# bepu/bepuphysics2

Hardware: NVIDIA H100
Metric: constraint-iterations/sec (solver+integrator) (higher is better)
Workload: dtype f32

## Files before the change

### bepuphysics2_b200/csrc/bepu_layout_kernels.h

```cpp
#pragma once
#include "bepu_device_types.h"

namespace bepucuda {

void launch_split_bodies(const void* raw, int body_count, const BodyBuffers& B, cudaStream_t s);
void launch_merge_bodies(void* raw, int body_count, const BodyBuffers& B, cudaStream_t s);
struct TransposeDesc {
    int32_t* src_refs;
    float* src_prestep;
    float* src_impulses;
    const int32_t* map;
    int32_t src_count;
    int32_t bodies, prestep_rows, impulse_rows;
    int32_t src_bundle_base;
    int32_t flags;
    const int32_t* features_old;
    const int32_t* features_new;
};
constexpr int32_t kDescResidentImpulses = 1, kDescRedistribute = 2;
enum { kTransposeRefs = 1, kTransposePrestep = 2, kTransposeImpulses = 4 };
void launch_transpose_in_all(const DeviceTypeBatch* tbs, const TransposeDesc* descs, const WorkItem* work, int work_count, int W, int what, cudaStream_t s);
void launch_transpose_out_all(const DeviceTypeBatch* tbs, const TransposeDesc* descs, const WorkItem* work, int work_count, int W, int what, cudaStream_t s);
void launch_fill_i32(int32_t* p, size_t n, int32_t v, cudaStream_t s);
void launch_redistribute_impulses(const DeviceTypeBatch* tbs, const TransposeDesc* descs, const WorkItem* work, int work_count, cudaStream_t s);
// ... 5 lines not shown
    size_t bytes;
};
void launch_batched_copy(const CopyChunk* chunks, int chunk_count, cudaStream_t s);
void launch_ownership_pass1(const DeviceTypeBatch* tbs, const WorkItem* work, int work_count, const int32_t* bodies_per_type, int sync_batch_count, int body_count,
                            int32_t* first_batch, int32_t* sync_refcount, unsigned long long* sync_mask, int32_t* error_flag, cudaStream_t s);
void launch_ownership_rest(const DeviceTypeBatch* tbs, const WorkItem* work, int work_count, const int32_t* bodies_per_type, int body_count, const int32_t* first_batch,
                           const int32_t* sync_refcount, const unsigned long long* sync_mask, uint8_t* constrained, const int32_t* kinematics, int kinematic_count,
                           int32_t* error_flag, const TransposeDesc* descs, int W, int32_t* source_bundle_flags, cudaStream_t s);
void launch_shard_barrier(const ShardPeers& peers, const FrameParams* fp, uint32_t exchange_index, int32_t* error_flag, cudaStream_t s);

void launch_fill_peer_masks(const int32_t* refs, uint32_t* peer_masks, size_t count, const uint8_t* body_masks, int rank, cudaStream_t s);
void launch_boundary_flags(const WorkRecord* records, int count, const int32_t* bodies_per_type, long long peer_delta, uint8_t* flags, cudaStream_t s);

void launch_pack_ref_rows(const WorkRecord* records, int count, int32_t* rows, cudaStream_t s);

constexpr int kLaunchPdl = 1, kLaunchPrefetchRows = 2, kLaunchIntegratorExtensions = 4;
struct ShardLaunch {
    ShardPeers peers;
    long long peer_delta;
    ShardStage stage;
};
struct SolverLaunchers {
    void (*constraint_stage)(int stage, const WorkRecord* records, const int32_t* ref_rows, int work_count, const BodyBuffers& B, const FrameParams* fp, int launch_flags,
                             const ShardLaunch* shard, cudaStream_t s);
    void (*kinematic_stage)(int stage, const int32_t* kinematics, int count, const BodyBuffers& B, const FrameParams* fp, int launch_flags, cudaStream_t s);
    void (*final_pose)(const BodyBuffers& B, const FrameParams* fp, int launch_flags, cudaStream_t s);
};
const SolverLaunchers* get_launchers_bepu_fast();
const SolverLaunchers* get_launchers_bepu_strict();

}
// ... 1 lines not shown
```

### bepuphysics2_b200/csrc/bepu_solver_kernels.cu

```cuda
#include <atomic>
#include "bepu_solver_kernels.cuh"
#include "bepu_layout_kernels.h"

namespace BEPU_NS {

using StageLauncher = void(const WorkRecord* records, const int32_t* ref_rows, int work_count, const BodyBuffers& B, const FrameParams* fp, int launch_flags,
                           const ShardLaunch* shard, cudaStream_t s);
StageLauncher launch_stage_warm_start_first, launch_stage_warm_start, launch_stage_solve;

#ifndef BEPU_DEEP_MINB
#define BEPU_DEEP_MINB 12
#endif
constexpr int kDeepBatchBundles = 2150;
template <auto Kernel, class... Args>
static void launch_stage_kernel(int work_count, int launch_flags, cudaStream_t s, Args... args) {
    static std::atomic<bool> carveout_set[64] = {};
    int device = 0;
    cudaGetDevice(&device);
    if (!carveout_set[device & 63]) {
        cudaFuncSetAttribute(Kernel, cudaFuncAttributePreferredSharedMemoryCarveout, cudaSharedmemCarveoutMaxShared);
        carveout_set[device & 63] = true;
    }
    const unsigned blocks = (unsigned)(((size_t)work_count * 32 + kStageBlockThreads - 1) / kStageBlockThreads);
    cudaLaunchConfig_t cfg{};
    cfg.gridDim = dim3(blocks);
    cfg.blockDim = dim3(kStageBlockThreads);
    cfg.stream = s;
    cudaLaunchAttribute attr[1];
    attr[0].id = cudaLaunchAttributeProgrammaticStreamSerialization;
    attr[0].val.programmaticStreamSerializationAllowed = 1;
    cfg.attrs = attr;
    cfg.numAttrs = (launch_flags & bepucuda::kLaunchPdl) ? 1 : 0;
    cudaLaunchKernelEx(&cfg, Kernel, args...);
}
template <int STAGE, int MINB, bool kExt>
static void launch_stage_instance(const WorkRecord* records, const int32_t* ref_rows, int work_count, const BodyBuffers& B, const FrameParams* fp, int launch_flags, const ShardLaunch* shard,
                                  cudaStream_t s) {
    const int flags = (launch_flags & bepucuda::kLaunchPrefetchRows) ? kStagePrefetchRows : 0;
    if (!shard) launch_stage_kernel<constraint_stage_kernel<STAGE, MINB, kExt>>(work_count, launch_flags, s, records, ref_rows, work_count, B, fp, flags);
    else if constexpr (STAGE != kStageIncremental)
        launch_stage_kernel<constraint_stage_kernel_sharded<STAGE, MINB, kExt>>(work_count, launch_flags, s, records, ref_rows, work_count, B, fp, flags, shard->peers, shard->peer_delta,
                                                                               shard->stage);
}
template <int STAGE, int MINB>
static void launch_stage_variant(const WorkRecord* records, const int32_t* ref_rows, int work_count, const BodyBuffers& B, const FrameParams* fp, int launch_flags, const ShardLaunch* shard,
                                 cudaStream_t s) {
    if constexpr (STAGE == kStageWarmStartFirst || STAGE == kStageWarmStart) {
        if (launch_flags & bepucuda::kLaunchIntegratorExtensions) return launch_stage_instance<STAGE, MINB, true>(records, ref_rows, work_count, B, fp, launch_flags, shard, s);
    }
    launch_stage_instance<STAGE, MINB, false>(records, ref_rows, work_count, B, fp, launch_flags, shard, s);
}
template <int STAGE>
static void launch_stage_t(const WorkRecord* records, const int32_t* ref_rows, int work_count, const BodyBuffers& B, const FrameParams* fp, int launch_flags, const ShardLaunch* shard, cudaStream_t s) {
    if constexpr (STAGE != kStageIncremental) {
        if (work_count >= kDeepBatchBundles) return launch_stage_variant<STAGE, BEPU_DEEP_MINB>(records, ref_rows, work_count, B, fp, launch_flags, shard, s);
    }
    launch_stage_variant<STAGE, 1>(records, ref_rows, work_count, B, fp, launch_flags, shard, s);
}

#if BEPU_UNIT == 0
void launch_stage_warm_start_first(const WorkRecord* records, const int32_t* ref_rows, int work_count, const BodyBuffers& B, const FrameParams* fp, int launch_flags, const ShardLaunch* shard, cudaStream_t s) {
    launch_stage_t<kStageWarmStartFirst>(records, ref_rows, work_count, B, fp, launch_flags, shard, s);
}
#elif BEPU_UNIT == 1
void launch_stage_warm_start(const WorkRecord* records, const int32_t* ref_rows, int work_count, const BodyBuffers& B, const FrameParams* fp, int launch_flags, const ShardLaunch* shard, cudaStream_t s) {
    launch_stage_t<kStageWarmStart>(records, ref_rows, work_count, B, fp, launch_flags, shard, s);
}
#elif BEPU_UNIT == 2
void launch_stage_solve(const WorkRecord* records, const int32_t* ref_rows, int work_count, const BodyBuffers& B, const FrameParams* fp, int launch_flags, const ShardLaunch* shard, cudaStream_t s) {
    launch_stage_t<kStageSolve>(records, ref_rows, work_count, B, fp, launch_flags, shard, s);
}
#elif BEPU_UNIT == 3
// ... 36 lines not shown
```

### bepuphysics2_b200/csrc/bepu_solver_kernels.cuh

```cuda
#pragma once
#include "bepu_contacts.cuh"
#include "bepu_joints_more.cuh"
#include "bepu_integration.cuh"
#include "bepu_device_types.h"

namespace BEPU_NS {

using namespace bepucuda;

struct F8 { float a, b, c, d, e, f, g, h; };
#define BEPU_BODY_LD "ld.global.L1::no_allocate.L2::cache_hint.v4.f32"
#define BEPU_BODY_ST "st.global.L1::no_allocate.L2::cache_hint.v4.f32"
BEPU_DI uint64_t l2_evict_last_policy() {
    uint64_t policy;
    asm("createpolicy.fractional.L2::evict_last.b64 %0, 1.0;" : "=l"(policy));
    return policy;
}
BEPU_DI F8 ld256(const float4* p) {
    F8 r;
    asm volatile(BEPU_BODY_LD " {%0,%1,%2,%3}, [%8], %9;\n\t" BEPU_BODY_LD " {%4,%5,%6,%7}, [%8+16], %9;"
                 : "=f"(r.a), "=f"(r.b), "=f"(r.c), "=f"(r.d), "=f"(r.e), "=f"(r.f), "=f"(r.g), "=f"(r.h)
                 : "l"(p), "l"(l2_evict_last_policy())
                 : "memory");
    return r;
// ... 29 lines not shown
    if (flags & kIntegrateAccelerations) {
        const F8 a = ld256(accelerations + 2 * (size_t)idx);
        linearAcceleration = {a.a, a.b, a.c};
        angularAcceleration = {a.e, a.f, a.g};
    }
    integrate_velocity_extensions(v, (flags & kIntegrateAccelerations) != 0, linearAcceleration, angularAcceleration, dt, (flags & kIntegratePointGravity) != 0, position, center,
                                  attractorDt);
    return v;
}
BEPU_DI void apply_velocity_extensions(const FrameParams& fp, uint32_t idx, V3 position, float dt, float attractorDt, Velocity& v) {
    const float4* accelerations = reinterpret_cast<const float4*>((unsigned long long)fp.accelerations[0] | ((unsigned long long)fp.accelerations[1] << 32));
    v = integrate_velocity_extensions_at(fp.integrate_extensions, accelerations, idx, v.lin, v.ang, dt, position, V3{fp.attractor_center[0], fp.attractor_center[1], fp.attractor_center[2]},
                                         attractorDt);
}

template <int STAGE, bool NeedsPose, bool kExt>
BEPU_DI void warm_start_body(uint32_t enc, const BodyBuffers& B, const FrameParams& fp, BodyState& b, Velocity& v) {
    const uint32_t idx = enc & kRefIndexMask;
    if (enc & kRefIntegrateBit) {
        Inertia local;
        load_inertia(B.inertia_local, idx, local);
        load_pose(B.pose, idx, b.pos, b.q);
        b.inertia.inv_mass = local.inv_mass;
        if (STAGE == kStageWarmStart) {
            b.pos = b.pos + v.lin * fp.dt;
            Q4 previousOrientation = b.q;
            b.q = integrate_orientation(b.q, v.ang, fp.dt * 0.5f);
            b.inertia.t = rotate_inverse_inertia(local.t, b.q);
            if (fp.angular_mode == 1) integrate_angular_conserve_momentum(previousOrientation, local.t, b.inertia.t, v.ang);
            else if (fp.angular_mode == 2) integrate_angular_gyroscopic(b.q, local.t, v.ang, fp.dt);
            store_pose(B.pose, idx, b.pos, b.q);
        } else {
            b.inertia.t = rotate_inverse_inertia(local.t, b.q);
            if (fp.angular_mode == 1) {
                Q4 previousOrientation = integrate_orientation(b.q, v.ang, fp.dt * -0.5f);
                integrate_angular_conserve_momentum(previousOrientation, local.t, b.inertia.t, v.ang);
            } else if (fp.angular_mode == 2) {
// ... 6 lines not shown
    } else {
        load_inertia(B.inertia_world, idx, b.inertia);
        if (NeedsPose) load_pose(B.pose, idx, b.pos, b.q);
        if (STAGE == kStageWarmStartFirst && fp.angular_mode != 0 && (enc & kRefBundleIntegratesBit) && !(enc & kRefKinematicBit)) {
            Inertia local;
            load_inertia(B.inertia_local, idx, local);
            V3 pos;
            Q4 q;
            load_pose(B.pose, idx, pos, q);
            if (fp.angular_mode == 1) integrate_angular_conserve_momentum(integrate_orientation(q, v.ang, fp.dt * -0.5f), local.t, b.inertia.t, v.ang);
            else integrate_angular_gyroscopic(q, local.t, v.ang, fp.dt);
        }
    }
}
template <int STAGE, bool NeedsPose, bool kExt>
BEPU_DI void gather_for_warm_start(uint32_t enc, const BodyBuffers& B, const FrameParams& fp, BodyState& b, Velocity& v) {
    load_velocity(B.velocity, enc & kRefIndexMask, v);
    warm_start_body<STAGE, NeedsPose, kExt>(enc, B, fp, b, v);
}

template <class T, class PR, class AR> BEPU_DI void call_warm_start(const BodyState* b, PR p, AR a, Velocity* v) {
    if constexpr (T::kNeedsPose) T::warm_start(b, p, a, v);
    else if constexpr (T::kBodies == 2) T::warm_start(b[0].inertia, b[1].inertia, p, a, v[0], v[1]);
    else T::warm_start(b[0].inertia, p, a, v[0]);
}
template <class T, class PR, class AR> BEPU_DI void call_solve(const BodyState* b, float dt, float inverseDt, PR p, AR a, Velocity* v) {
    if constexpr (T::kNeedsPose) T::solve(b, dt, inverseDt, p, a, v);
    else if constexpr (T::kBodies == 2) T::solve(b[0].inertia, b[1].inertia, dt, inverseDt, p, a, v[0], v[1]);
    else T::solve(b[0].inertia, dt, inverseDt, p, a, v[0]);
}
template <class T> BEPU_DI void call_incremental(float dt, const Velocity* v, float* p) {
    if constexpr (T::kIncremental) {
        if constexpr (T::kBodies == 2) T::incremental_update(dt, v[0], v[1], p);
// ... 4 lines not shown
BEPU_DI uint32_t ldg_nc_u32(const void* p) {
    uint32_t v;
    asm volatile("ld.global.nc.u32 %0, [%1];" : "=r"(v) : "l"(p));
    return v;
}
BEPU_DI void push_record(float4* const* arrays, uint32_t mask, uint32_t idx, float a, float b, float c, float d, float e, float f, float g, float h) {
    while (mask) {
        const int q = __ffs((int)mask) - 1;
        mask &= mask - 1u;
        float4* dst = arrays[q] + 2 * (size_t)idx;
        dst[0] = make_float4(a, b, c, d);
        dst[1] = make_float4(e, f, g, h);
    }
}
template <class T, int STAGE, bool kSharded, bool kExt, class PR, class AR>
BEPU_DI void run_lane(const int32_t* refs, PR p, AR a, float* p_rw, uint32_t enc0, uint32_t enc1, const BodyBuffers& B, const FrameParams& fp, const ShardPeers* peers = nullptr,
                      long long peer_delta = 0) {
    constexpr int NB = T::kBodies;
    uint32_t enc[NB];
    enc[0] = enc0;
    if constexpr (NB > 1) enc[1] = enc1;
#pragma unroll
    for (int s = 2; s < NB; ++s) enc[s] = (uint32_t)__ldg(refs + s * kLanes);
    uint32_t push_to[kSharded ? NB : 1];
    if constexpr (kSharded) {
#pragma unroll
        for (int s = 0; s < NB; ++s) push_to[s] = peer_delta != 0 ? ldg_nc_u32(refs + peer_delta + s * kLanes) : 0u;
    }
    if ((int32_t)enc[0] == kRefEmpty) return;
    BodyState b[NB];
    Velocity v[NB];
    if constexpr (STAGE == kStageIncremental) {
#pragma unroll
        for (int s = 0; s < NB; ++s) load_velocity(B.velocity, enc[s] & kRefIndexMask, v[s]);
        call_incremental<T>(fp.dt, v, p_rw);
    } else if constexpr (STAGE == kStageSolve) {
#pragma unroll
        for (int s = 0; s < NB; ++s) {
            const uint32_t idx = enc[s] & kRefIndexMask;
            load_velocity(B.velocity, idx, v[s]);
            load_inertia(B.inertia_world, idx, b[s].inertia);
            if (T::kNeedsPose) load_pose(B.pose, idx, b[s].pos, b[s].q);
        }
        rows_ready(p);
        call_solve<T>(b, fp.dt, fp.inverse_dt, p, a, v);
#pragma unroll
        for (int s = 0; s < NB; ++s)
            if (!(enc[s] & kRefKinematicBit)) {
                store_velocity(B.velocity, enc[s] & kRefIndexMask, v[s]);
                if constexpr (kSharded) {
                    const uint32_t mask = push_to[s];
                    if (mask) push_record(peers->velocity, mask, enc[s] & kRefIndexMask, v[s].lin.x, v[s].lin.y, v[s].lin.z, 0.0f, v[s].ang.x, v[s].ang.y, v[s].ang.z, 0.0f);
                }
            }
    } else {
#pragma unroll
        for (int s = 0; s < NB; ++s) gather_for_warm_start<STAGE, T::kNeedsPose, kExt>(enc[s], B, fp, b[s], v[s]);
        rows_ready(p);
        call_warm_start<T>(b, p, a, v);
#pragma unroll
        for (int s = 0; s < NB; ++s)
            if (!(enc[s] & kRefKinematicBit)) {
                const uint32_t idx = enc[s] & kRefIndexMask;
                store_velocity(B.velocity, idx, v[s]);
                if constexpr (kSharded) {
                    const uint32_t mask = push_to[s];
                    if (mask) {
                        push_record(peers->velocity, mask, idx, v[s].lin.x, v[s].lin.y, v[s].lin.z, 0.0f, v[s].ang.x, v[s].ang.y, v[s].ang.z, 0.0f);
                        if (enc[s] & kRefIntegrateBit) {
                            const Inertia& in = b[s].inertia;
                            push_record(peers->inertia_world, mask, idx, in.t.xx, in.t.yx, in.t.yy, in.t.zx, in.t.zy, in.t.zz, in.inv_mass, 0.0f);
                            if (STAGE == kStageWarmStart) push_record(peers->pose, mask, idx, b[s].q.x, b[s].q.y, b[s].q.z, b[s].q.w, b[s].pos.x, b[s].pos.y, b[s].pos.z, 0.0f);
                        }
                    }
                }
            }
    }
}
template <class T, int STAGE, class PR, class AR>
BEPU_DI void run_lane(const int32_t* refs, PR p, AR a, float* p_rw, uint32_t enc0, uint32_t enc1, const BodyBuffers& B, const FrameParams& fp) {
    run_lane<T, STAGE, false, false>(refs, p, a, p_rw, enc0, enc1, B, fp);
}

BEPU_DI int4 ldg_nc_v4(const void* p) {
    int4 v;
    asm volatile("ld.global.nc.v4.s32 {%0,%1,%2,%3}, [%4];" : "=r"(v.x), "=r"(v.y), "=r"(v.z), "=r"(v.w) : "l"(p));
    return v;
}
BEPU_DI WorkRecord load_record(const WorkRecord* r) {
    const int4 lo = ldg_nc_v4(r), hi = ldg_nc_v4(reinterpret_cast<const int4*>(r) + 1);
    WorkRecord w;
    w.refs = reinterpret_cast<int32_t*>((unsigned long long)(unsigned int)lo.x | ((unsigned long long)(unsigned int)lo.y << 32));
    w.prestep = reinterpret_cast<float*>((unsigned long long)(unsigned int)lo.z | ((unsigned long long)(unsigned int)lo.w << 32));
    w.impulses = reinterpret_cast<float*>((unsigned long long)(unsigned int)hi.x | ((unsigned long long)(unsigned int)hi.y << 32));
    w.type_id = hi.z;
    w.live_lanes = hi.w;
    return w;
}

#define BEPU_CONTACT_TYPES(X)                                                                                                     \
    X(0, ConvexOneBody<1>) X(1, ConvexOneBody<2>) X(2, ConvexOneBody<3>) X(3, ConvexOneBody<4>)                                   \
    X(4, ConvexTwoBody<1>) X(5, ConvexTwoBody<2>) X(6, ConvexTwoBody<3>) X(7, ConvexTwoBody<4>)                                   \
    X(8, NonconvexOneBody<2>) X(9, NonconvexOneBody<3>) X(10, NonconvexOneBody<4>)                                                \
    X(15, NonconvexTwoBody<2>) X(16, NonconvexTwoBody<3>) X(17, NonconvexTwoBody<4>)

template <int STAGE, bool kSharded, bool kExt, class PR, class AR>
BEPU_DI void run_bundle_rows(const WorkRecord& rec, int lane, PR p, AR a, uint32_t enc0, uint32_t enc1, const BodyBuffers& B, const FrameParams& fp, const ShardPeers* peers = nullptr,
                             long long peer_delta = 0) {
    const int32_t* refs = rec.refs + lane;
    float* p_rw = rec.prestep + lane;
    switch (rec.type_id) {
#define BEPU_CASE(ID, T) \
    case ID: run_lane<T, STAGE, kSharded, kExt>(refs, p, a, p_rw, enc0, enc1, B, fp, peers, peer_delta); break;
        BEPU_CONTACT_TYPES(BEPU_CASE)
        BEPU_JOINT_TYPES(BEPU_CASE)
        BEPU_JOINT_TYPES_MORE(BEPU_CASE)
#undef BEPU_CASE
        default: break;
    }
}
template <int STAGE, class PR, class AR>
BEPU_DI void run_bundle_rows(const WorkRecord& rec, int lane, PR p, AR a, uint32_t enc0, uint32_t enc1, const BodyBuffers& B, const FrameParams& fp) {
    run_bundle_rows<STAGE, false, false>(rec, lane, p, a, enc0, enc1, B, fp);
}
template <int STAGE>
BEPU_DI void run_bundle(const WorkRecord& rec, int lane, uint32_t enc0, uint32_t enc1, const BodyBuffers& B, const FrameParams& fp) {
    run_bundle_rows<STAGE>(rec, lane, GlobalRows{rec.prestep + lane}, GlobalAcc{rec.impulses + lane}, enc0, enc1, B, fp);
}
template <int STAGE> BEPU_DI void run_bundle(const WorkRecord& rec, int lane, const BodyBuffers& B, const FrameParams& fp) {
    const uint32_t enc0 = ldg_nc_u32(rec.refs + lane), enc1 = ldg_nc_u32(rec.refs + kLanes + lane);
    run_bundle<STAGE>(rec, lane, enc0, enc1, B, fp);
}

struct StageRowCounts { uint8_t prestep[64], impulses[64]; };
__host__ __device__ constexpr StageRowCounts make_stage_row_counts() {
    StageRowCounts c{};
#define BEPU_ROWS(ID, T) c.prestep[ID] = (uint8_t)T::kPrestepRows; c.impulses[ID] = (uint8_t)T::kImpulseRows;
    BEPU_CONTACT_TYPES(BEPU_ROWS)
    BEPU_JOINT_TYPES(BEPU_ROWS)
    BEPU_JOINT_TYPES_MORE(BEPU_ROWS)
#undef BEPU_ROWS
    return c;
}
__constant__ StageRowCounts kStageRowCounts = make_stage_row_counts();
constexpr int kStageSlabRows = 48;
constexpr int kStageSlabBytes = kStageSlabRows * kLanes * 4;

BEPU_DI uint32_t smem_u32(const void* p) { return (uint32_t)__cvta_generic_to_shared(p); }
BEPU_DI void mbar_init(uint32_t bar, uint32_t count) {
    asm volatile("mbarrier.init.shared::cta.b64 [%0], %1;" ::"r"(bar), "r"(count) : "memory");
    asm volatile("fence.mbarrier_init.release.cluster;" ::: "memory");
    asm volatile("fence.proxy.async.shared::cta;" ::: "memory");
// ... 3 lines not shown
    uint64_t policy;
    asm volatile("createpolicy.fractional.L2::evict_first.b64 %0, 1.0;" : "=l"(policy));
    return policy;
}
BEPU_DI void bulk_copy_g2s(uint32_t dst, const void* src, uint32_t bytes, uint32_t bar, uint64_t policy) {
    asm volatile("cp.async.bulk.shared::cluster.global.mbarrier::complete_tx::bytes.L2::cache_hint [%0], [%1], %2, [%3], %4;" ::"r"(dst), "l"(src), "r"(bytes), "r"(bar),
                 "l"(policy)
                 : "memory");
}

#ifndef BEPU_STAGE_BLOCK_THREADS
#define BEPU_STAGE_BLOCK_THREADS 64
#endif
constexpr int kStageBlockThreads = BEPU_STAGE_BLOCK_THREADS;

constexpr int kStagePrefetchRows = 1;
BEPU_DI void shard_announce(const ShardPeers& peers, int lane) {
    if (lane < peers.rank_count && lane != peers.rank)
        asm volatile("red.release.sys.global.add.u64 [%0], 1;" ::"l"(peers.flags[lane] + kShardCounterSlot + peers.rank) : "memory");
}
BEPU_DI void shard_wait(const ShardPeers& peers, int lane, uint32_t solve_index, uint32_t exchange_point, int32_t* error_flag) {
    if (lane < peers.rank_count && lane != peers.rank) {
        const unsigned long long* mine = peers.flags[peers.rank];
        const unsigned long long* targets = mine + kShardTargetSlot + (size_t)lane * kShardMaxExchanges;
        const unsigned long long want = (unsigned long long)solve_index * targets[kShardMaxExchanges - 1] + targets[exchange_point];
        unsigned long long seen;
        unsigned int spins = 0;
        do {
            asm volatile("ld.acquire.sys.global.u64 %0, [%1];" : "=l"(seen) : "l"(mine + kShardCounterSlot + lane) : "memory");
        } while (seen < want && ++spins < 100000000u);
        if (seen < want) atomicExch(error_flag, 5);
    }
    __syncwarp();
}
template <int STAGE, bool kSharded, bool kExt>
BEPU_DI void constraint_stage_body(const WorkRecord* __restrict__ records, const int32_t* __restrict__ ref_rows, int work_count, const BodyBuffers& B, const FrameParams* __restrict__ fpp, int flags, const ShardPeers* peers,
                                   long long peer_delta, const ShardStage* shard = nullptr) {
    constexpr bool kStaged = STAGE != kStageIncremental;
    constexpr int kWarps = kStageBlockThreads / 32;
    __shared__ __align__(128) float slab[kStaged ? kWarps * kStageSlabRows * kLanes : 1];
    __shared__ __align__(8) unsigned long long bars[kWarps];
    const int warp_in_block = threadIdx.x >> 5;
    const int global_warp = (blockIdx.x * kStageBlockThreads + threadIdx.x) >> 5;
    const int lane = threadIdx.x & 31;
    WorkRecord rec{};
    uint32_t enc0 = (uint32_t)kRefEmpty, enc1 = 0;
    const int warp = global_warp;
    const bool active = warp < work_count;
    const uint32_t slab_addr = kStaged ? smem_u32(slab) + warp_in_block * kStageSlabBytes : 0;
    const uint32_t bar = smem_u32(&bars[warp_in_block]);
    const bool early_rows = kStaged && (flags & kStagePrefetchRows);
    uint32_t prestep_bytes = 0, impulse_bytes = 0;
    if (active) {
        rec = load_record(records + warp);
        if constexpr (kStaged) {
            prestep_bytes = kStageRowCounts.prestep[rec.type_id] * (kLanes * 4);
            impulse_bytes = kStageRowCounts.impulses[rec.type_id] * (kLanes * 4);
            if (lane == 0) {
                mbar_init(bar, 1);
                if (early_rows) {
                    const uint64_t policy = l2_evict_first_policy();
                    mbar_expect_tx(bar, prestep_bytes + impulse_bytes);
                    bulk_copy_g2s(slab_addr, rec.prestep, prestep_bytes, bar, policy);
                    bulk_copy_g2s(slab_addr + prestep_bytes, rec.impulses, impulse_bytes, bar, policy);
                }
            }
        }
        enc0 = ldg_nc_u32(ref_rows + (size_t)warp * (2 * kLanes) + lane);
        enc1 = ldg_nc_u32(ref_rows + (size_t)warp * (2 * kLanes) + kLanes + lane);
    }
    const FrameParams fp = *fpp;
    asm volatile("griddepcontrol.wait;" ::: "memory");
    asm volatile("griddepcontrol.launch_dependents;");
    bool boundary = false;
    if constexpr (kSharded) {
        boundary = active && (rec.live_lanes & kRecordBoundaryBit) != 0;
        if (boundary && shard->exchange_index > 0) shard_wait(*peers, lane, fp.shard_solve_index, shard->exchange_index - 1u, shard->error_flag);
    }
    if (!active) return;
    if constexpr (kStaged) {
        if (!early_rows && lane == 0) {
            const uint64_t policy = l2_evict_first_policy();
            mbar_expect_tx(bar, prestep_bytes + impulse_bytes);
            bulk_copy_g2s(slab_addr, rec.prestep, prestep_bytes, bar, policy);
            bulk_copy_g2s(slab_addr + prestep_bytes, rec.impulses, impulse_bytes, bar, policy);
        }
        __syncwarp();
        run_bundle_rows<STAGE, kSharded, kExt>(rec, lane, StagedRows{slab_addr + lane * 4, bar, 0u}, StagedAcc{slab_addr + prestep_bytes + lane * 4, rec.impulses + lane}, enc0, enc1, B, fp,
                                         peers, boundary ? peer_delta : 0);
        if constexpr (kSharded) {
            if (boundary) {
                __syncwarp();
                shard_announce(*peers, lane);
            }
        }
    } else {
        run_bundle<STAGE>(rec, lane, enc0, enc1, B, fp);
    }
}

template <int STAGE, int MINB, bool kExt>
__global__ void __launch_bounds__(kStageBlockThreads, MINB) constraint_stage_kernel(const WorkRecord* __restrict__ records, const int32_t* __restrict__ ref_rows, int work_count, BodyBuffers B, const FrameParams* __restrict__ fpp, int flags) {
    constraint_stage_body<STAGE, false, kExt>(records, ref_rows, work_count, B, fpp, flags, nullptr, 0);
}
template <int STAGE, int MINB, bool kExt>
__global__ void __launch_bounds__(kStageBlockThreads, MINB)
constraint_stage_kernel_sharded(const WorkRecord* __restrict__ records, const int32_t* __restrict__ ref_rows, int work_count, BodyBuffers B, const FrameParams* __restrict__ fpp, int flags, const __grid_constant__ ShardPeers peers,
                                long long peer_delta, const __grid_constant__ ShardStage shard) {
    constraint_stage_body<STAGE, true, kExt>(records, ref_rows, work_count, B, fpp, flags, &peers, peer_delta, &shard);
}

#if BEPU_UNIT == 3
template <int STAGE, bool kExt> BEPU_DI void run_kinematic(int i, const int32_t* kinematics, const BodyBuffers& B, const FrameParams& fp) {
    const uint32_t idx = (uint32_t)kinematics[i];
    Velocity v;
    load_velocity(B.velocity, idx, v);
    V3 pos{0.0f, 0.0f, 0.0f};
    Q4 q;
    if (STAGE == kStageKinematic) {
        load_pose(B.pose, idx, pos, q);
        pos = pos + v.lin * fp.dt;
        q = integrate_orientation(q, v.ang, fp.dt * 0.5f);
        store_pose(B.pose, idx, pos, q);
    }
// ... 64 lines not shown
```

### bepuphysics2_b200/csrc/bepucuda_api.cu

```cuda
#include <algorithm>
#include <cmath>
#include <cstring>
#include <string>
#include <vector>

#include "../../include/bepucuda.h"
#include "bepu_layout_kernels.h"
#include "bepu_coloring.h"
#include "bepu_bounds.h"

using namespace bepucuda;

namespace bepucuda {

static TypeInfo make_contact(int bodies, int prestep, int impulses, int contacts, const char* name) {
    TypeInfo t{};
    t.bodies = bodies; t.prestep_rows = prestep; t.impulse_rows = impulses; t.incremental = 1; t.name = name;
    const int body_rw = 13 + 6;
    t.solve_bytes = 4 * (prestep + 2 * impulses + bodies + bodies * body_rw);
    t.warm_start_bytes = 4 * (prestep + impulses + bodies + bodies * body_rw);
    t.incremental_bytes = 4 * (prestep + contacts + bodies + 6 * bodies);
    return t;
}
static TypeInfo make_joint(int bodies, int prestep, int impulses, int solve_r, int solve_w, int ws_r, int ws_w, const char* name) {
// ... 18 lines not shown
        add(10, make_contact(1, 32, 12, 4, "Contact4NonconvexOneBody"));
        add(15, make_contact(2, 21, 6, 2, "Contact2Nonconvex")); add(16, make_contact(2, 28, 9, 3, "Contact3Nonconvex"));
        add(17, make_contact(2, 35, 12, 4, "Contact4Nonconvex"));
#define BEPU_REGISTER_JOINTS
#include "bepu_joint_registry.inc"
#undef BEPU_REGISTER_JOINTS
    }
};
static const Registry& registry() {
    static Registry r;
    return r;
}
const TypeInfo* get_type_info(int type_id) {
    if (type_id < 0 || type_id >= 64 || !registry().present[type_id]) return nullptr;
    return &registry().types[type_id];
}

struct DeviceBuffer {
    void* ptr = nullptr;
    size_t capacity = 0;
    cudaError_t reserve(size_t bytes) {
        if (bytes <= capacity) return cudaSuccess;
        if (ptr) cudaFree(ptr);
        ptr = nullptr;
        capacity = 0;
        size_t want = bytes + bytes / 4 + 256;
        cudaError_t e = cudaMalloc(&ptr, want);
        if (e == cudaSuccess) capacity = want;
        return e;
    }
// ... 42 lines not shown
    float* raw_impulses;
    size_t refs_bytes, prestep_bytes, impulse_bytes;
    std::vector<int32_t> host_refs;
    std::vector<int> device_tbs;
    int32_t* raw_features_old = nullptr;
    int32_t* raw_features_new = nullptr;
    size_t feature_bytes = 0;
    bool resident_impulses = false, redistribute = false;
};

struct StageOp {
    int32_t stage;
    int32_t work_begin;
    int32_t work_count;
    int32_t exchange;
};
constexpr int32_t kNoExchange = -1, kRankBarrier = -2;

}

struct bepucuda_ctx {
    bepucuda_config cfg{};
    int device = 0;
    cudaStream_t stream = nullptr;
    cudaEvent_t ev_solve_begin = nullptr, ev_solve_end = nullptr, ev_up_begin = nullptr, ev_up_end = nullptr, ev_down_begin = nullptr, ev_down_end = nullptr;
    bool up_open = false, have_solve = false, have_down = false, have_up = false;
    std::string error;
    const SolverLaunchers* launchers = nullptr;

    std::vector<int32_t> iterations{1};
// ... 13 lines not shown
    DeviceBuffer raw_bodies, pose, velocity, inertia_local, inertia_world, constrained, first_batch, sync_refcount, sync_mask;
    BodyBuffers B{};

    int W = 8;
    int batch_count = 0;
    bool constraints_open = false, constraints_ready = false, data_dirty = false, descs_dirty = false;
    std::vector<SourceTypeBatch> sources;
    ChunkArena raw_arena, pinned_arena;
    DeviceBuffer record_table, ref_rows, source_bundle_flags, refs32, prestep32, impulses32, tb_table, tdesc_table, work_table, map_table, bodies_per_type, kinematics_dev, frame_params_dev, error_dev;
    std::vector<DeviceTypeBatch> tbs;
    std::vector<TransposeDesc> tdescs;
    std::vector<WorkItem> work;
    std::vector<int32_t> bundle_live;
    std::vector<WorkRecord> records;
    std::vector<std::pair<int, int>> batch_work;
    bool peer_mode = false;
    ShardPeers peers{};
    DeviceBuffer shard_flags, peer32, body_masks_dev, boundary_flags_dev;
    uint32_t shard_solve_index = 0;
    std::vector<int> boundary_count;
    std::vector<uint8_t> body_masks;
    size_t refs_words = 0;
    std::vector<void*> opened_ipc;
    std::vector<int32_t> global_first_batch;
    std::vector<uint8_t> global_constrained;
    uint32_t exchange_counter = 0;
    uint32_t exchanges_per_solve = 0;
    int inc_work_begin = 0, inc_work_count = 0;
    int all_work_count = 0;
    int sync_batch_count = 0, fallback_levels = 0;
// ... 98 lines not shown
}

void invalidate_graph(bepucuda_ctx* ctx) {
    if (ctx->graph_exec) cudaGraphExecDestroy(ctx->graph_exec);
    if (ctx->graph) cudaGraphDestroy(ctx->graph);
    ctx->graph_exec = nullptr;
    ctx->graph = nullptr;
    ctx->graph_valid = false;
}

bool integrator_extensions(const bepucuda_ctx* ctx) { return ctx->accelerations_count >= 0 || ctx->point_gravity; }

bool rows_prefetchable(const StageOp* previous, const StageOp& op) {
    return op.stage != kStageIncremental && previous != nullptr && previous->stage != kStageIncremental &&
           !(previous->stage <= kStageSolve && previous->work_begin == op.work_begin);
}

struct StageEvents {
    const std::vector<cudaEvent_t>& events;
    std::vector<int>& launched;
};

void issue_stage_sequence(bepucuda_ctx* ctx, cudaStream_t s, int64_t* launches, const StageEvents* profile = nullptr) {
    const WorkRecord* records = ctx->record_table.as<WorkRecord>();
    const int32_t* ref_rows = ctx->ref_rows.as<int32_t>();
    const FrameParams* fp = ctx->frame_params_dev.as<FrameParams>();
    const int32_t* kin = ctx->kinematics_dev.as<int32_t>();
    ShardLaunch shard{ctx->peers, (long long)(ctx->peer32.as<int32_t>() - ctx->refs32.as<int32_t>()), {0, ctx->error_dev.as<int32_t>()}};
    int64_t n = 0;
    const StageOp* previous = nullptr;
    uint32_t exchange_index = 0;
    const int extensions = integrator_extensions(ctx) ? kLaunchIntegratorExtensions : 0;
    for (size_t i = 0; i < ctx->program.size(); ++i) {
        const StageOp& op = ctx->program[i];
        const bool barrier = op.exchange == kRankBarrier;
        if (barrier || (op.stage == kStageFinalPose ? ctx->B.count > 0 : op.work_count > 0)) {
            if (profile) cudaEventRecord(profile->events[2 * i], s);
            if (barrier) {
                launch_shard_barrier(ctx->peers, fp, exchange_index, ctx->error_dev.as<int32_t>(), s);
            } else if (op.stage <= kStageIncremental) {
                shard.stage.exchange_index = exchange_index;
                const int flags = (profile ? 0 : kLaunchPdl | (rows_prefetchable(previous, op) ? kLaunchPrefetchRows : 0)) | extensions;
                ctx->launchers->constraint_stage(op.stage, records + op.work_begin, ref_rows + (size_t)op.work_begin * 64, op.work_count, ctx->B, fp, flags,
                                                 op.exchange == kNoExchange ? nullptr : &shard, s);
            } else if (op.stage <= kStageKinematic) {
                ctx->launchers->kinematic_stage(op.stage, kin, op.work_count, ctx->B, fp, extensions, s);
            } else {
                ctx->launchers->final_pose(ctx->B, fp, extensions, s);
            }
            if (profile) {
                cudaEventRecord(profile->events[2 * i + 1], s);
                profile->launched[i] = 1;
            }
            if (!barrier) previous = &op;
            ++n;
        }
        if (op.exchange != kNoExchange) ++exchange_index;
// ... 5 lines not shown
    ctx->program.clear();
    const int substeps = (int)ctx->iterations.size();
    const int kin = (int)ctx->kinematics.size();
    const StageOp rank_barrier{kStageKinematic, 0, 0, kRankBarrier};
    for (int s = 0; s < substeps; ++s) {
        if (s > 0) {
            if (ctx->peer_mode) ctx->program.push_back(rank_barrier);
            if (ctx->inc_work_count > 0) ctx->program.push_back({kStageIncremental, ctx->inc_work_begin, ctx->inc_work_count, kNoExchange});
            if (kin > 0) ctx->program.push_back({kStageKinematic, 0, kin, kNoExchange});
        } else if (ctx->integ.integrate_velocity_for_kinematics && kin > 0) {
            ctx->program.push_back({kStageKinematicFirst, 0, kin, kNoExchange});
        }
        if (ctx->peer_mode) ctx->program.push_back(rank_barrier);
        for (size_t b = 0; b < ctx->batch_work.size(); ++b) {
            auto& bw = ctx->batch_work[b];
            if (bw.second > 0 || (ctx->peer_mode && (int)b < ctx->sync_batch_count)) ctx->program.push_back({s == 0 ? kStageWarmStartFirst : kStageWarmStart, bw.first, bw.second, ctx->peer_mode ? (int)b : kNoExchange});
        }
        for (int it = 0; it < ctx->iterations[s]; ++it)
            for (size_t b = 0; b < ctx->batch_work.size(); ++b) {
                auto& bw = ctx->batch_work[b];
                if (bw.second > 0 || (ctx->peer_mode && (int)b < ctx->sync_batch_count)) ctx->program.push_back({kStageSolve, bw.first, bw.second, ctx->peer_mode ? (int)b : kNoExchange});
            }
    }
    if (ctx->peer_mode) ctx->program.push_back(rank_barrier);
    ctx->program.push_back({kStageFinalPose, 0, ctx->body_count, kNoExchange});
}

int upload_program(bepucuda_ctx* ctx) {
    build_program(ctx);
    if (ctx->peer_mode) {
        std::vector<unsigned long long> targets((size_t)kShardMaxExchanges, 0ull);
        unsigned long long arrived = 0;
        size_t e = 0;
        for (const StageOp& op : ctx->program) {
            if (op.exchange == kNoExchange) continue;
            if (e + 1 >= (size_t)kShardMaxExchanges) return fail(ctx, BEPUCUDA_ERR_BAD_STATE, "peer sharding: more than 4095 exchange points per solve");
// ... 519 lines not shown
    CK(ctx->refs32.reserve(refs_floats * 4 + 1024));
    ctx->refs_words = refs_floats;
    CK(ctx->prestep32.reserve(prestep_floats * 4 + 4));
    CK(ctx->impulses32.reserve(impulse_floats * 4 + 4));
    CK(ctx->map_table.reserve(maps.size() * 4 + 4));
    for (size_t i = 0; i < ctx->tbs.size(); ++i) {
        ctx->tbs[i].refs = ctx->refs32.as<int32_t>() + ro[i];
        ctx->tbs[i].prestep = ctx->prestep32.as<float>() + po[i];
        ctx->tbs[i].impulses = ctx->impulses32.as<float>() + io[i];
        ctx->tdescs[i].map = map_offset[i] == SIZE_MAX ? nullptr : ctx->map_table.as<int32_t>() + map_offset[i];
    }

    ctx->work.clear();
    ctx->bundle_live.clear();
    ctx->batch_work.clear();
    auto live_in_bundle = [&](int tb, int k) {
        if (map_offset[tb] == SIZE_MAX) return std::max(0, std::min(32, ctx->tdescs[tb].src_count - k * 32));
        int n = 0;
        for (int l = 0; l < 32; ++l) n += maps[map_offset[tb] + (size_t)k * 32 + l] >= 0;
        return n;
    };
    for (auto& list : batch_tbs) {
        const int begin = (int)ctx->work.size();
        for (int tb : list)
            for (int k = 0; k < ctx->tbs[tb].bundle_count; ++k) { ctx->work.push_back({tb, k}); ctx->bundle_live.push_back(live_in_bundle(tb, k)); }
        ctx->batch_work.push_back({begin, (int)ctx->work.size() - begin});
    }
    ctx->all_work_count = (int)ctx->work.size();
    ctx->inc_work_begin = (int)ctx->work.size();
    for (size_t tb = 0; tb < ctx->tbs.size(); ++tb)
        if (get_type_info(ctx->tbs[tb].type_id)->incremental)
            for (int k = 0; k < ctx->tbs[tb].bundle_count; ++k) { ctx->work.push_back({(int)tb, k}); ctx->bundle_live.push_back(live_in_bundle((int)tb, k)); }
    ctx->inc_work_count = (int)ctx->work.size() - ctx->inc_work_begin;

    ctx->records.resize(ctx->work.size());
    for (size_t i = 0; i < ctx->work.size(); ++i) {
        const WorkItem& w = ctx->work[i];
        const DeviceTypeBatch& tb = ctx->tbs[w.type_batch];
        const TypeInfo* t = get_type_info(tb.type_id);
        WorkRecord r{};
        r.refs = tb.refs + (size_t)w.bundle * t->bodies * 32;
// ... 615 lines not shown
```

Baseline: 2.007 billion.

## Prefetch body state before grid dependency wait and specialize contact-only batch kernels

Adds a prefetch that loads body inertia and pose for the first two bodies of each lane before griddepcontrol.wait, when the previous stage did not touch the same batch. This overlaps body gathers with the tail of the previous kernel. It also adds contact-only kernel variants that drop the joint switch cases and use higher min-blocks launch bounds, meant to lower register pressure and raise occupancy. The cost is extra registers to hold the early body state and more template instantiations. There is also a risk of reading body data before the previous kernel's writes are visible, which the bodies_prefetchable check is meant to prevent.

```diff
diff --git a/bepuphysics2_b200/csrc/bepu_layout_kernels.h b/bepuphysics2_b200/csrc/bepu_layout_kernels.h
--- a/bepuphysics2_b200/csrc/bepu_layout_kernels.h
+++ b/bepuphysics2_b200/csrc/bepu_layout_kernels.h
@@ -43,7 +43,7 @@
 
 void launch_pack_ref_rows(const WorkRecord* records, int count, int32_t* rows, cudaStream_t s);
 
-constexpr int kLaunchPdl = 1, kLaunchPrefetchRows = 2, kLaunchIntegratorExtensions = 4;
+constexpr int kLaunchPdl = 1, kLaunchPrefetchRows = 2, kLaunchIntegratorExtensions = 4, kLaunchContactsOnly = 8, kLaunchPrefetchBodies = 16;
 struct ShardLaunch {
     ShardPeers peers;
     long long peer_delta;
diff --git a/bepuphysics2_b200/csrc/bepu_solver_kernels.cu b/bepuphysics2_b200/csrc/bepu_solver_kernels.cu
--- a/bepuphysics2_b200/csrc/bepu_solver_kernels.cu
+++ b/bepuphysics2_b200/csrc/bepu_solver_kernels.cu
@@ -12,6 +12,12 @@
 #define BEPU_DEEP_MINB 12
 #endif
 constexpr int kDeepBatchBundles = 2150;
+#ifndef BEPU_CONTACT_MINB
+#define BEPU_CONTACT_MINB 10
+#endif
+#ifndef BEPU_CONTACT_SOLVE_MINB
+#define BEPU_CONTACT_SOLVE_MINB 12
+#endif
 template <auto Kernel, class... Args>
 static void launch_stage_kernel(int work_count, int launch_flags, cudaStream_t s, Args... args) {
     static std::atomic<bool> carveout_set[64] = {};
@@ -33,29 +39,31 @@
     cfg.numAttrs = (launch_flags & bepucuda::kLaunchPdl) ? 1 : 0;
     cudaLaunchKernelEx(&cfg, Kernel, args...);
 }
-template <int STAGE, int MINB, bool kExt>
+template <int STAGE, int MINB, bool kExt, bool kContacts>
 static void launch_stage_instance(const WorkRecord* records, const int32_t* ref_rows, int work_count, const BodyBuffers& B, const FrameParams* fp, int launch_flags, const ShardLaunch* shard,
                                   cudaStream_t s) {
-    const int flags = (launch_flags & bepucuda::kLaunchPrefetchRows) ? kStagePrefetchRows : 0;
-    if (!shard) launch_stage_kernel<constraint_stage_kernel<STAGE, MINB, kExt>>(work_count, launch_flags, s, records, ref_rows, work_count, B, fp, flags);
-    else if constexpr (STAGE != kStageIncremental)
+    const int flags = ((launch_flags & bepucuda::kLaunchPrefetchRows) ? kStagePrefetchRows : 0) | ((launch_flags & bepucuda::kLaunchPrefetchBodies) ? kStagePrefetchBodies : 0);
+    if (!shard) launch_stage_kernel<constraint_stage_kernel<STAGE, MINB, kExt, kContacts>>(work_count, launch_flags, s, records, ref_rows, work_count, B, fp, flags);
+    else if constexpr (STAGE != kStageIncremental && !kContacts)
         launch_stage_kernel<constraint_stage_kernel_sharded<STAGE, MINB, kExt>>(work_count, launch_flags, s, records, ref_rows, work_count, B, fp, flags, shard->peers, shard->peer_delta,
                                                                                shard->stage);
 }
-template <int STAGE, int MINB>
+template <int STAGE, int MINB, bool kContacts>
 static void launch_stage_variant(const WorkRecord* records, const int32_t* ref_rows, int work_count, const BodyBuffers& B, const FrameParams* fp, int launch_flags, const ShardLaunch* shard,
                                  cudaStream_t s) {
     if constexpr (STAGE == kStageWarmStartFirst || STAGE == kStageWarmStart) {
-        if (launch_flags & bepucuda::kLaunchIntegratorExtensions) return launch_stage_instance<STAGE, MINB, true>(records, ref_rows, work_count, B, fp, launch_flags, shard, s);
+        if (launch_flags & bepucuda::kLaunchIntegratorExtensions) return launch_stage_instance<STAGE, MINB, true, kContacts>(records, ref_rows, work_count, B, fp, launch_flags, shard, s);
     }
-    launch_stage_instance<STAGE, MINB, false>(records, ref_rows, work_count, B, fp, launch_flags, shard, s);
+    launch_stage_instance<STAGE, MINB, false, kContacts>(records, ref_rows, work_count, B, fp, launch_flags, shard, s);
 }
 template <int STAGE>
 static void launch_stage_t(const WorkRecord* records, const int32_t* ref_rows, int work_count, const BodyBuffers& B, const FrameParams* fp, int launch_flags, const ShardLaunch* shard, cudaStream_t s) {
     if constexpr (STAGE != kStageIncremental) {
-        if (work_count >= kDeepBatchBundles) return launch_stage_variant<STAGE, BEPU_DEEP_MINB>(records, ref_rows, work_count, B, fp, launch_flags, shard, s);
+        if (work_count >= kDeepBatchBundles) return launch_stage_variant<STAGE, BEPU_DEEP_MINB, false>(records, ref_rows, work_count, B, fp, launch_flags, shard, s);
+        if (!shard && (launch_flags & bepucuda::kLaunchContactsOnly))
+            return launch_stage_variant<STAGE, STAGE == kStageSolve ? BEPU_CONTACT_SOLVE_MINB : BEPU_CONTACT_MINB, true>(records, ref_rows, work_count, B, fp, launch_flags, shard, s);
     }
-    launch_stage_variant<STAGE, 1>(records, ref_rows, work_count, B, fp, launch_flags, shard, s);
+    launch_stage_variant<STAGE, 1, false>(records, ref_rows, work_count, B, fp, launch_flags, shard, s);
 }
 
 #if BEPU_UNIT == 0
diff --git a/bepuphysics2_b200/csrc/bepu_solver_kernels.cuh b/bepuphysics2_b200/csrc/bepu_solver_kernels.cuh
--- a/bepuphysics2_b200/csrc/bepu_solver_kernels.cuh
+++ b/bepuphysics2_b200/csrc/bepu_solver_kernels.cuh
@@ -67,13 +67,26 @@
                                          attractorDt);
 }
 
+struct EarlyBodies {
+    uint32_t slots;
+    Inertia inertia[2];
+    V3 pos[2];
+    Q4 q[2];
+};
+
 template <int STAGE, bool NeedsPose, bool kExt>
-BEPU_DI void warm_start_body(uint32_t enc, const BodyBuffers& B, const FrameParams& fp, BodyState& b, Velocity& v) {
+BEPU_DI void warm_start_body(uint32_t enc, const BodyBuffers& B, const FrameParams& fp, bool early_slot, const EarlyBodies& early, int s, BodyState& b, Velocity& v) {
     const uint32_t idx = enc & kRefIndexMask;
     if (enc & kRefIntegrateBit) {
         Inertia local;
-        load_inertia(B.inertia_local, idx, local);
-        load_pose(B.pose, idx, b.pos, b.q);
+        if (early_slot) {
+            local = early.inertia[s];
+            b.pos = early.pos[s];
+            b.q = early.q[s];
+        } else {
+            load_inertia(B.inertia_local, idx, local);
+            load_pose(B.pose, idx, b.pos, b.q);
+        }
         b.inertia.inv_mass = local.inv_mass;
         if (STAGE == kStageWarmStart) {
             b.pos = b.pos + v.lin * fp.dt;
@@ -110,9 +123,9 @@
     }
 }
 template <int STAGE, bool NeedsPose, bool kExt>
-BEPU_DI void gather_for_warm_start(uint32_t enc, const BodyBuffers& B, const FrameParams& fp, BodyState& b, Velocity& v) {
+BEPU_DI void gather_for_warm_start(uint32_t enc, const BodyBuffers& B, const FrameParams& fp, bool early_slot, const EarlyBodies& early, int s, BodyState& b, Velocity& v) {
     load_velocity(B.velocity, enc & kRefIndexMask, v);
-    warm_start_body<STAGE, NeedsPose, kExt>(enc, B, fp, b, v);
+    warm_start_body<STAGE, NeedsPose, kExt>(enc, B, fp, early_slot, early, s, b, v);
 }
 
 template <class T, class PR, class AR> BEPU_DI void call_warm_start(const BodyState* b, PR p, AR a, Velocity* v) {
@@ -147,8 +160,8 @@
     }
 }
 template <class T, int STAGE, bool kSharded, bool kExt, class PR, class AR>
-BEPU_DI void run_lane(const int32_t* refs, PR p, AR a, float* p_rw, uint32_t enc0, uint32_t enc1, const BodyBuffers& B, const FrameParams& fp, const ShardPeers* peers = nullptr,
-                      long long peer_delta = 0) {
+BEPU_DI void run_lane(const int32_t* refs, PR p, AR a, float* p_rw, uint32_t enc0, uint32_t enc1, const BodyBuffers& B, const FrameParams& fp, const EarlyBodies& early,
+                      const ShardPeers* peers = nullptr, long long peer_delta = 0) {
     constexpr int NB = T::kBodies;
     uint32_t enc[NB];
     enc[0] = enc0;
@@ -172,8 +185,13 @@
         for (int s = 0; s < NB; ++s) {
             const uint32_t idx = enc[s] & kRefIndexMask;
             load_velocity(B.velocity, idx, v[s]);
-            load_inertia(B.inertia_world, idx, b[s].inertia);
-            if (T::kNeedsPose) load_pose(B.pose, idx, b[s].pos, b[s].q);
+            if (s < 2 && (early.slots >> s & 1u)) {
+                b[s].inertia = early.inertia[s & 1];
+                if (T::kNeedsPose) b[s].pos = early.pos[s & 1], b[s].q = early.q[s & 1];
+            } else {
+                load_inertia(B.inertia_world, idx, b[s].inertia);
+                if (T::kNeedsPose) load_pose(B.pose, idx, b[s].pos, b[s].q);
+            }
         }
         rows_ready(p);
         call_solve<T>(b, fp.dt, fp.inverse_dt, p, a, v);
@@ -188,7 +206,7 @@
             }
     } else {
 #pragma unroll
-        for (int s = 0; s < NB; ++s) gather_for_warm_start<STAGE, T::kNeedsPose, kExt>(enc[s], B, fp, b[s], v[s]);
+        for (int s = 0; s < NB; ++s) gather_for_warm_start<STAGE, T::kNeedsPose, kExt>(enc[s], B, fp, s < 2 && (early.slots >> s & 1u), early, s & 1, b[s], v[s]);
         rows_ready(p);
         call_warm_start<T>(b, p, a, v);
 #pragma unroll
@@ -210,10 +228,6 @@
             }
     }
 }
-template <class T, int STAGE, class PR, class AR>
-BEPU_DI void run_lane(const int32_t* refs, PR p, AR a, float* p_rw, uint32_t enc0, uint32_t enc1, const BodyBuffers& B, const FrameParams& fp) {
-    run_lane<T, STAGE, false, false>(refs, p, a, p_rw, enc0, enc1, B, fp);
-}
 
 BEPU_DI int4 ldg_nc_v4(const void* p) {
     int4 v;
@@ -237,38 +251,42 @@
     X(8, NonconvexOneBody<2>) X(9, NonconvexOneBody<3>) X(10, NonconvexOneBody<4>)                                                \
     X(15, NonconvexTwoBody<2>) X(16, NonconvexTwoBody<3>) X(17, NonconvexTwoBody<4>)
 
-template <int STAGE, bool kSharded, bool kExt, class PR, class AR>
-BEPU_DI void run_bundle_rows(const WorkRecord& rec, int lane, PR p, AR a, uint32_t enc0, uint32_t enc1, const BodyBuffers& B, const FrameParams& fp, const ShardPeers* peers = nullptr,
-                             long long peer_delta = 0) {
+template <int STAGE, bool kSharded, bool kExt, bool kContacts, class PR, class AR>
+BEPU_DI void run_bundle_rows(const WorkRecord& rec, int lane, PR p, AR a, uint32_t enc0, uint32_t enc1, const BodyBuffers& B, const FrameParams& fp, const EarlyBodies& early,
+                             const ShardPeers* peers = nullptr, long long peer_delta = 0) {
     const int32_t* refs = rec.refs + lane;
     float* p_rw = rec.prestep + lane;
-    switch (rec.type_id) {
 #define BEPU_CASE(ID, T) \
-    case ID: run_lane<T, STAGE, kSharded, kExt>(refs, p, a, p_rw, enc0, enc1, B, fp, peers, peer_delta); break;
-        BEPU_CONTACT_TYPES(BEPU_CASE)
-        BEPU_JOINT_TYPES(BEPU_CASE)
-        BEPU_JOINT_TYPES_MORE(BEPU_CASE)
+    case ID: run_lane<T, STAGE, kSharded, kExt>(refs, p, a, p_rw, enc0, enc1, B, fp, early, peers, peer_delta); break;
+    if constexpr (kContacts) {
+        switch (rec.type_id) {
+            BEPU_CONTACT_TYPES(BEPU_CASE)
+            default: break;
+        }
+    } else {
+        switch (rec.type_id) {
+            BEPU_CONTACT_TYPES(BEPU_CASE)
+            BEPU_JOINT_TYPES(BEPU_CASE)
+            BEPU_JOINT_TYPES_MORE(BEPU_CASE)
+            default: break;
+        }
+    }
 #undef BEPU_CASE
-        default: break;
-    }
-}
-template <int STAGE, class PR, class AR>
-BEPU_DI void run_bundle_rows(const WorkRecord& rec, int lane, PR p, AR a, uint32_t enc0, uint32_t enc1, const BodyBuffers& B, const FrameParams& fp) {
-    run_bundle_rows<STAGE, false, false>(rec, lane, p, a, enc0, enc1, B, fp);
 }
 template <int STAGE>
 BEPU_DI void run_bundle(const WorkRecord& rec, int lane, uint32_t enc0, uint32_t enc1, const BodyBuffers& B, const FrameParams& fp) {
-    run_bundle_rows<STAGE>(rec, lane, GlobalRows{rec.prestep + lane}, GlobalAcc{rec.impulses + lane}, enc0, enc1, B, fp);
+    run_bundle_rows<STAGE, false, false, false>(rec, lane, GlobalRows{rec.prestep + lane}, GlobalAcc{rec.impulses + lane}, enc0, enc1, B, fp, EarlyBodies{});
 }
 template <int STAGE> BEPU_DI void run_bundle(const WorkRecord& rec, int lane, const BodyBuffers& B, const FrameParams& fp) {
     const uint32_t enc0 = ldg_nc_u32(rec.refs + lane), enc1 = ldg_nc_u32(rec.refs + kLanes + lane);
     run_bundle<STAGE>(rec, lane, enc0, enc1, B, fp);
 }
 
-struct StageRowCounts { uint8_t prestep[64], impulses[64]; };
+struct StageRowCounts { uint8_t prestep[64], impulses[64], bodies[64], needs_pose[64]; };
 __host__ __device__ constexpr StageRowCounts make_stage_row_counts() {
     StageRowCounts c{};
-#define BEPU_ROWS(ID, T) c.prestep[ID] = (uint8_t)T::kPrestepRows; c.impulses[ID] = (uint8_t)T::kImpulseRows;
+#define BEPU_ROWS(ID, T) \
+    c.prestep[ID] = (uint8_t)T::kPrestepRows; c.impulses[ID] = (uint8_t)T::kImpulseRows; c.bodies[ID] = (uint8_t)T::kBodies; c.needs_pose[ID] = T::kNeedsPose ? 1 : 0;
     BEPU_CONTACT_TYPES(BEPU_ROWS)
     BEPU_JOINT_TYPES(BEPU_ROWS)
     BEPU_JOINT_TYPES_MORE(BEPU_ROWS)
@@ -302,7 +320,28 @@
 #endif
 constexpr int kStageBlockThreads = BEPU_STAGE_BLOCK_THREADS;
 
-constexpr int kStagePrefetchRows = 1;
+constexpr int kStagePrefetchRows = 1, kStagePrefetchBodies = 2;
+template <int STAGE, bool kContacts>
+BEPU_DI void load_early_bodies(int type_id, uint32_t enc0, uint32_t enc1, const BodyBuffers& B, EarlyBodies& e) {
+    if ((int32_t)enc0 == kRefEmpty) return;
+    const int bodies = kStageRowCounts.bodies[type_id];
+    const bool pose = !kContacts && kStageRowCounts.needs_pose[type_id];
+#pragma unroll
+    for (int s = 0; s < 2; ++s) {
+        const uint32_t enc = s == 0 ? enc0 : enc1;
+        const uint32_t idx = enc & kRefIndexMask;
+        if (s >= bodies) break;
+        if (STAGE == kStageSolve) {
+            load_inertia(B.inertia_world, idx, e.inertia[s]);
+            if (pose) load_pose(B.pose, idx, e.pos[s], e.q[s]);
+            e.slots |= 1u << s;
+        } else if (enc & kRefIntegrateBit) {
+            load_inertia(B.inertia_local, idx, e.inertia[s]);
+            load_pose(B.pose, idx, e.pos[s], e.q[s]);
+            e.slots |= 1u << s;
+        }
+    }
+}
 BEPU_DI void shard_announce(const ShardPeers& peers, int lane) {
     if (lane < peers.rank_count && lane != peers.rank)
         asm volatile("red.release.sys.global.add.u64 [%0], 1;" ::"l"(peers.flags[lane] + kShardCounterSlot + peers.rank) : "memory");
@@ -321,7 +360,7 @@
     }
     __syncwarp();
 }
-template <int STAGE, bool kSharded, bool kExt>
+template <int STAGE, bool kSharded, bool kExt, bool kContacts, bool kEarlyBodies>
 BEPU_DI void constraint_stage_body(const WorkRecord* __restrict__ records, const int32_t* __restrict__ ref_rows, int work_count, const BodyBuffers& B, const FrameParams* __restrict__ fpp, int flags, const ShardPeers* peers,
                                    long long peer_delta, const ShardStage* shard = nullptr) {
     constexpr bool kStaged = STAGE != kStageIncremental;
@@ -339,6 +378,7 @@
     const uint32_t bar = smem_u32(&bars[warp_in_block]);
     const bool early_rows = kStaged && (flags & kStagePrefetchRows);
     uint32_t prestep_bytes = 0, impulse_bytes = 0;
+    EarlyBodies early{};
     if (active) {
         rec = load_record(records + warp);
         if constexpr (kStaged) {
@@ -356,6 +396,9 @@
         }
         enc0 = ldg_nc_u32(ref_rows + (size_t)warp * (2 * kLanes) + lane);
         enc1 = ldg_nc_u32(ref_rows + (size_t)warp * (2 * kLanes) + kLanes + lane);
+        if constexpr (kStaged && kEarlyBodies) {
+            if (flags & kStagePrefetchBodies) load_early_bodies<STAGE, kContacts>(rec.type_id, enc0, enc1, B, early);
+        }
     }
     const FrameParams fp = *fpp;
     asm volatile("griddepcontrol.wait;" ::: "memory");
@@ -374,8 +417,8 @@
             bulk_copy_g2s(slab_addr + prestep_bytes, rec.impulses, impulse_bytes, bar, policy);
         }
         __syncwarp();
-        run_bundle_rows<STAGE, kSharded, kExt>(rec, lane, StagedRows{slab_addr + lane * 4, bar, 0u}, StagedAcc{slab_addr + prestep_bytes + lane * 4, rec.impulses + lane}, enc0, enc1, B, fp,
-                                         peers, boundary ? peer_delta : 0);
+        run_bundle_rows<STAGE, kSharded, kExt, kContacts>(rec, lane, StagedRows{slab_addr + lane * 4, bar, 0u}, StagedAcc{slab_addr + prestep_bytes + lane * 4, rec.impulses + lane}, enc0,
+                                                          enc1, B, fp, early, peers, boundary ? peer_delta : 0);
         if constexpr (kSharded) {
             if (boundary) {
                 __syncwarp();
@@ -387,15 +430,15 @@
     }
 }
 
-template <int STAGE, int MINB, bool kExt>
+template <int STAGE, int MINB, bool kExt, bool kContacts>
 __global__ void __launch_bounds__(kStageBlockThreads, MINB) constraint_stage_kernel(const WorkRecord* __restrict__ records, const int32_t* __restrict__ ref_rows, int work_count, BodyBuffers B, const FrameParams* __restrict__ fpp, int flags) {
-    constraint_stage_body<STAGE, false, kExt>(records, ref_rows, work_count, B, fpp, flags, nullptr, 0);
+    constraint_stage_body<STAGE, false, kExt, kContacts, MINB == 1 || kContacts>(records, ref_rows, work_count, B, fpp, flags, nullptr, 0);
 }
 template <int STAGE, int MINB, bool kExt>
 __global__ void __launch_bounds__(kStageBlockThreads, MINB)
 constraint_stage_kernel_sharded(const WorkRecord* __restrict__ records, const int32_t* __restrict__ ref_rows, int work_count, BodyBuffers B, const FrameParams* __restrict__ fpp, int flags, const __grid_constant__ ShardPeers peers,
                                 long long peer_delta, const __grid_constant__ ShardStage shard) {
-    constraint_stage_body<STAGE, true, kExt>(records, ref_rows, work_count, B, fpp, flags, &peers, peer_delta, &shard);
+    constraint_stage_body<STAGE, true, kExt, false, false>(records, ref_rows, work_count, B, fpp, flags, &peers, peer_delta, &shard);
 }
 
 #if BEPU_UNIT == 3
diff --git a/bepuphysics2_b200/csrc/bepucuda_api.cu b/bepuphysics2_b200/csrc/bepucuda_api.cu
--- a/bepuphysics2_b200/csrc/bepucuda_api.cu
+++ b/bepuphysics2_b200/csrc/bepucuda_api.cu
@@ -56,6 +56,10 @@
 const TypeInfo* get_type_info(int type_id) {
     if (type_id < 0 || type_id >= 64 || !registry().present[type_id]) return nullptr;
     return &registry().types[type_id];
+}
+static bool is_contact_type(int type_id) {
+    const TypeInfo* t = get_type_info(type_id);
+    return t && t->incremental != 0;
 }
 
 struct DeviceBuffer {
@@ -128,6 +132,7 @@
     int32_t work_begin;
     int32_t work_count;
     int32_t exchange;
+    int32_t contacts_only;
 };
 constexpr int32_t kNoExchange = -1, kRankBarrier = -2;
 
@@ -171,6 +176,7 @@
     std::vector<int32_t> bundle_live;
     std::vector<WorkRecord> records;
     std::vector<std::pair<int, int>> batch_work;
+    std::vector<int32_t> batch_contacts_only;
     bool peer_mode = false;
     ShardPeers peers{};
     DeviceBuffer shard_flags, peer32, body_masks_dev, boundary_flags_dev;
@@ -299,6 +305,9 @@
 bool rows_prefetchable(const StageOp* previous, const StageOp& op) {
     return op.stage != kStageIncremental && previous != nullptr && previous->stage != kStageIncremental &&
            !(previous->stage <= kStageSolve && previous->work_begin == op.work_begin);
+}
+bool bodies_prefetchable(const StageOp* previous, const StageOp& op) {
+    return op.stage <= kStageSolve && previous != nullptr && !(previous->stage <= kStageWarmStart && previous->work_begin == op.work_begin);
 }
 
 struct StageEvents {
@@ -325,7 +334,8 @@
                 launch_shard_barrier(ctx->peers, fp, exchange_index, ctx->error_dev.as<int32_t>(), s);
             } else if (op.stage <= kStageIncremental) {
                 shard.stage.exchange_index = exchange_index;
-                const int flags = (profile ? 0 : kLaunchPdl | (rows_prefetchable(previous, op) ? kLaunchPrefetchRows : 0)) | extensions;
+                const int prefetch = (rows_prefetchable(previous, op) ? kLaunchPrefetchRows : 0) | (bodies_prefetchable(previous, op) ? kLaunchPrefetchBodies : 0);
+                const int flags = (profile ? 0 : kLaunchPdl | prefetch) | extensions | (op.contacts_only ? kLaunchContactsOnly : 0);
                 ctx->launchers->constraint_stage(op.stage, records + op.work_begin, ref_rows + (size_t)op.work_begin * 64, op.work_count, ctx->B, fp, flags,
                                                  op.exchange == kNoExchange ? nullptr : &shard, s);
             } else if (op.stage <= kStageKinematic) {
@@ -361,12 +371,14 @@
         if (ctx->peer_mode) ctx->program.push_back(rank_barrier);
         for (size_t b = 0; b < ctx->batch_work.size(); ++b) {
             auto& bw = ctx->batch_work[b];
-            if (bw.second > 0 || (ctx->peer_mode && (int)b < ctx->sync_batch_count)) ctx->program.push_back({s == 0 ? kStageWarmStartFirst : kStageWarmStart, bw.first, bw.second, ctx->peer_mode ? (int)b : kNoExchange});
+            if (bw.second > 0 || (ctx->peer_mode && (int)b < ctx->sync_batch_count))
+                ctx->program.push_back({s == 0 ? kStageWarmStartFirst : kStageWarmStart, bw.first, bw.second, ctx->peer_mode ? (int)b : kNoExchange, ctx->batch_contacts_only[b]});
         }
         for (int it = 0; it < ctx->iterations[s]; ++it)
             for (size_t b = 0; b < ctx->batch_work.size(); ++b) {
                 auto& bw = ctx->batch_work[b];
-                if (bw.second > 0 || (ctx->peer_mode && (int)b < ctx->sync_batch_count)) ctx->program.push_back({kStageSolve, bw.first, bw.second, ctx->peer_mode ? (int)b : kNoExchange});
+                if (bw.second > 0 || (ctx->peer_mode && (int)b < ctx->sync_batch_count))
+                    ctx->program.push_back({kStageSolve, bw.first, bw.second, ctx->peer_mode ? (int)b : kNoExchange, ctx->batch_contacts_only[b]});
             }
     }
     if (ctx->peer_mode) ctx->program.push_back(rank_barrier);
@@ -916,6 +928,7 @@
     ctx->work.clear();
     ctx->bundle_live.clear();
     ctx->batch_work.clear();
+    ctx->batch_contacts_only.clear();
     auto live_in_bundle = [&](int tb, int k) {
         if (map_offset[tb] == SIZE_MAX) return std::max(0, std::min(32, ctx->tdescs[tb].src_count - k * 32));
         int n = 0;
@@ -924,9 +937,13 @@
     };
     for (auto& list : batch_tbs) {
         const int begin = (int)ctx->work.size();
-        for (int tb : list)
+        bool contacts_only = true;
+        for (int tb : list) {
+            contacts_only = contacts_only && is_contact_type(ctx->tbs[tb].type_id);
             for (int k = 0; k < ctx->tbs[tb].bundle_count; ++k) { ctx->work.push_back({tb, k}); ctx->bundle_live.push_back(live_in_bundle(tb, k)); }
+        }
         ctx->batch_work.push_back({begin, (int)ctx->work.size() - begin});
+        ctx->batch_contacts_only.push_back(contacts_only ? 1 : 0);
     }
     ctx->all_work_count = (int)ctx->work.size();
     ctx->inc_work_begin = (int)ctx->work.size();
```

Result: faster. 2.196 billion (median of 6 runs) (+9.4%).
